# OmerMersin/video-stab

Measured on AMD Instinct MI355X. Metric: stabilized frames/sec @1080p (whole job; warp-stage HBM GB/s in roofline), higher is better.
Workload: dtype u8

## Files before the change

video-stab_amd/csrc/k_pyr.hip:

```cpp
#include "vs_common.h"

namespace vsd {
namespace {

constexpr int NT = 256;
constexpr int RPB = 4;

__global__ __launch_bounds__(NT) void pyr_down_kernel(const uint8_t* __restrict__ src_, size_t sstride,
                                                      int sw, int sh, uint8_t* __restrict__ dst_,
                                                      size_t dstride, int dw, int dh) {
    const uint8_t* __restrict__ src = src_;
    uint8_t* __restrict__ dst = dst_;
    const int x = blockIdx.x * blockDim.x + threadIdx.x;
    if (x >= dw) return;
    int xi[5];
#pragma unroll
    for (int k = 0; k < 5; k++) xi[k] = reflect101(2 * x + k - 2, sw);
    for (int y = blockIdx.y * RPB; y < min((int)(blockIdx.y + 1) * RPB, dh); y++) {
        int col[5];
#pragma unroll
        for (int j = 0; j < 5; j++) {
            const uint8_t* s = src + (size_t)reflect101(2 * y + j - 2, sh) * sstride;
            col[j] = s[xi[2]] * 6 + (s[xi[1]] + s[xi[3]]) * 4 + s[xi[0]] + s[xi[4]];
        }
        dst[(size_t)y * dstride + x] = (uint8_t)((col[2] * 6 + (col[1] + col[3]) * 4 + col[0] + col[4] + 128) >> 8);
    }
}

__global__ __launch_bounds__(NT) void scharr_kernel(const uint8_t* __restrict__ src_, size_t sstride, int w,
                                                    int h, int16_t* __restrict__ dst_) {
    const uint8_t* __restrict__ src = src_;
    int16_t* __restrict__ dst = dst_;
    const int x = blockIdx.x * blockDim.x + threadIdx.x;
    if (x >= w) return;
    for (int y = blockIdx.y * RPB; y < min((int)(blockIdx.y + 1) * RPB, h); y++) {
    const uint8_t* r0 = src + (size_t)(y > 0 ? y - 1 : h > 1 ? 1 : 0) * sstride;
    const uint8_t* r1 = src + (size_t)y * sstride;
    const uint8_t* r2 = src + (size_t)(y < h - 1 ? y + 1 : h > 1 ? h - 2 : 0) * sstride;
    const int xm = x > 0 ? x - 1 : (w > 1 ? 1 : 0);
    const int xp = x < w - 1 ? x + 1 : (w > 1 ? w - 2 : 0);
    const int a_m = (r0[xm] + r2[xm]) * 3 + r1[xm] * 10;
    const int a_p = (r0[xp] + r2[xp]) * 3 + r1[xp] * 10;
    const int b_m = r2[xm] - r0[xm];
    const int b_c = r2[x] - r0[x];
    const int b_p = r2[xp] - r0[xp];
    short2 o;
    o.x = (short)(a_p - a_m);
    o.y = (short)((b_p + b_m) * 3 + b_c * 10);
    *reinterpret_cast<short2*>(dst + ((size_t)y * w + x) * 2) = o;
    }
}

constexpr int FT_W = 64, FT_H = 16;
constexpr int FT_PITCH = 72;
constexpr int FT_ROWS = FT_H + 4;

template <bool DER, bool DOWN>
__global__ __launch_bounds__(NT) void pyr_level_kernel(const ImgPair* __restrict__ sch, const ImgPair* __restrict__ pyr, size_t sstride,
                                                       int w, int h, size_t dstride, int dw, int dh) {
    static_assert(DER || DOWN, "a level launch produces something");
    __shared__ __attribute__((aligned(16))) uint8_t tile[FT_ROWS * FT_PITCH];
    const uint8_t* __restrict__ src = static_cast<const uint8_t*>((DER ? sch : pyr)[blockIdx.z].src);
    const int tid = threadIdx.x;
    const int x0 = blockIdx.x * FT_W, y0 = blockIdx.y * FT_H;
    const bool inside = x0 >= 4 && y0 >= 2 && x0 + FT_W + 4 <= w && y0 + FT_H + 2 <= h && (sstride & 3) == 0 && ((uintptr_t)src & 3) == 0;
    if (inside) {
        constexpr int ND = (FT_ROWS * (FT_PITCH / 4) + NT - 1) / NT;
        uint32_t v[ND];
#pragma unroll
        for (int k = 0; k < ND; k++) {
            const int i = min(tid + NT * k, FT_ROWS * (FT_PITCH / 4) - 1);
            const int r = i / (FT_PITCH / 4), c4 = i - r * (FT_PITCH / 4);
            v[k] = *reinterpret_cast<const uint32_t*>(src + (size_t)(y0 - 2 + r) * sstride + (x0 - 4) + 4 * c4);
        }
#pragma unroll
        for (int k = 0; k < ND; k++)
            if (tid + NT * k < FT_ROWS * (FT_PITCH / 4)) reinterpret_cast<uint32_t*>(tile)[tid + NT * k] = v[k];
    } else if (tid < 3 * FT_PITCH) {
        constexpr int NB = (FT_ROWS + 2) / 3;
        const int c = tid % FT_PITCH, r0 = tid / FT_PITCH;
        const uint8_t* col = src + reflect101(x0 - 4 + c, w);
        size_t off[NB];
#pragma unroll
        for (int k = 0; k < NB; k++) off[k] = (size_t)reflect101(y0 - 2 + min(r0 + 3 * k, FT_ROWS - 1), h) * sstride;
        uint8_t v[NB];
#pragma unroll
        for (int k = 0; k < NB; k++) v[k] = col[off[k]];
#pragma unroll
        for (int k = 0; k < NB; k++)
            if (r0 + 3 * k < FT_ROWS) tile[(r0 + 3 * k) * FT_PITCH + c] = v[k];
    }
    __syncthreads();
    const uint32_t* T = reinterpret_cast<const uint32_t*>(tile);
    if (DER) {
        int16_t* __restrict__ der = static_cast<int16_t*>(sch[blockIdx.z].dst);
        const int r = tid >> 4, c = (tid & 15) * 4;
        const int y = y0 + r, x = x0 + c;
        if (y < h && x < w) {
            int t[3][6];
#pragma unroll
            for (int j = 0; j < 3; j++) {
                const uint32_t* q = T + (r + 1 + j) * (FT_PITCH / 4) + (c >> 2);
                const uint32_t lo = q[0], mid = q[1], hi = q[2];
                t[j][0] = lo >> 24;
                t[j][1] = mid & 255u; t[j][2] = (mid >> 8) & 255u; t[j][3] = (mid >> 16) & 255u; t[j][4] = mid >> 24;
                t[j][5] = hi & 255u;
            }
            int a[6], b[6];
#pragma unroll
            for (int k = 0; k < 6; k++) {
                a[k] = (t[0][k] + t[2][k]) * 3 + t[1][k] * 10;
                b[k] = t[2][k] - t[0][k];
            }
            uint32_t o[4];
#pragma unroll
            for (int k = 0; k < 4; k++) {
                const int dx = a[k + 2] - a[k], dy = (b[k + 2] + b[k]) * 3 + b[k + 1] * 10;
                o[k] = ((uint32_t)dx & 0xFFFFu) | ((uint32_t)dy << 16);
            }
            int16_t* d = der + ((size_t)y * w + x) * 2;
            if (x + 3 < w && (((uintptr_t)d) & 15) == 0) {
                *reinterpret_cast<uint4*>(d) = make_uint4(o[0], o[1], o[2], o[3]);
            } else {
                for (int k = 0; k < 4 && x + k < w; k++) reinterpret_cast<uint32_t*>(d)[k] = o[k];
            }
        }
    }
    if (DOWN) {
        uint8_t* __restrict__ dst = static_cast<uint8_t*>(pyr[blockIdx.z].dst);
        const int xo = (x0 >> 1) + (tid & 31), yo = (y0 >> 1) + (tid >> 5);
        if (xo < dw && yo < dh) {
            const int o = 2 * (tid & 31) + 2, sh = o & 3;
            const uint32_t* q = T + 2 * (tid >> 5) * (FT_PITCH / 4) + (o >> 2);
            int col[5];
#pragma unroll
            for (int j = 0; j < 5; j++) {
                const uint32_t lo = q[j * (FT_PITCH / 4)], hi = q[j * (FT_PITCH / 4) + 1];
                const uint32_t four = __builtin_amdgcn_alignbyte(hi, lo, sh);
                const uint32_t fifth = (hi >> (8 * sh)) & 255u;
                col[j] = (int)__builtin_amdgcn_udot4(four, 0x04060401u, fifth, false);
            }
            dst[(size_t)yo * dstride + xo] = (uint8_t)((col[2] * 6 + (col[1] + col[3]) * 4 + col[0] + col[4] + 128) >> 8);
        }
    }
}

}

int launch_pyr_level_batch(const ImgPair* d_scharr_pairs, const ImgPair* d_pyr_pairs, int items, size_t sstride, int w, int h,
                           size_t dstride, hipStream_t st) {
    if ((!d_scharr_pairs && !d_pyr_pairs) || items < 1 || items > 65535 || w <= 0 || h <= 0 || h > 65535) {
        set_last_error("pyr_level_batch: invalid argument");
        return VS_ERR_INVALID_ARG;
    }
    const int dw = (w + 1) / 2, dh = (h + 1) / 2;
    dim3 grid((w + FT_W - 1) / FT_W, (h + FT_H - 1) / FT_H, items);
    if (!d_scharr_pairs)
        hipLaunchKernelGGL((pyr_level_kernel<false, true>), grid, dim3(NT), 0, st, d_scharr_pairs, d_pyr_pairs, sstride, w, h, dstride, dw, dh);
    else if (d_pyr_pairs)
        hipLaunchKernelGGL((pyr_level_kernel<true, true>), grid, dim3(NT), 0, st, d_scharr_pairs, d_pyr_pairs, sstride, w, h, dstride, dw, dh);
    else hipLaunchKernelGGL((pyr_level_kernel<true, false>), grid, dim3(NT), 0, st, d_scharr_pairs, d_pyr_pairs, sstride, w, h, dstride, dw, dh);
    VS_HIP_TRY(hipGetLastError());
    return VS_OK;
}

int launch_pyr_down(const uint8_t* d_src, size_t sstride, int sw, int sh, uint8_t* d_dst,
                    size_t dstride, hipStream_t st) {
    if (!d_src || !d_dst || sw <= 0 || sh <= 0 || sh > 131070) {
        set_last_error("pyr_down: invalid argument");
        return VS_ERR_INVALID_ARG;
    }
    const int dw = (sw + 1) / 2, dh = (sh + 1) / 2;
    dim3 grid((dw + NT - 1) / NT, (dh + RPB - 1) / RPB);
    hipLaunchKernelGGL(pyr_down_kernel, grid, dim3(NT), 0, st, d_src, sstride, sw, sh, d_dst, dstride, dw, dh);
    VS_HIP_TRY(hipGetLastError());
    return VS_OK;
}

int launch_scharr(const uint8_t* d_src, size_t sstride, int w, int h, int16_t* d_dst, hipStream_t st) {
    if (!d_src || !d_dst || w <= 0 || h <= 0 || h > 65535) {
        set_last_error("scharr: invalid argument");
        return VS_ERR_INVALID_ARG;
    }
    dim3 grid((w + NT - 1) / NT, (h + RPB - 1) / RPB);
    hipLaunchKernelGGL(scharr_kernel, grid, dim3(NT), 0, st, d_src, sstride, w, h, d_dst);
    VS_HIP_TRY(hipGetLastError());
    return VS_OK;
}

}
```

video-stab_amd/csrc/vs_api.cpp:

```cpp
#include <cmath>
#include <cstring>
#include <mutex>
#include <vector>

#include "launchers.h"
#include "vs_common.h"

namespace vsd {

static thread_local std::string g_last_error;
void set_last_error(const std::string& msg) { g_last_error = msg; }
const char* get_last_error() { return g_last_error.c_str(); }

int ensure_device() {
    int n = 0;
    hipError_t e = hipGetDeviceCount(&n);
    if (e != hipSuccess || n <= 0) {
        set_last_error(std::string("no HIP device: ") + (e != hipSuccess ? hipGetErrorString(e) : "count is 0") +
                       " (libvideo-stab has no CPU fallback)");
        return VS_ERR_NO_DEVICE;
    }
    return VS_OK;
}

// ... 149 lines not shown
int vs_dev_sync(void) {
    VS_TRY(ensure_device());
    VS_HIP_TRY(hipDeviceSynchronize());
    return VS_OK;
}
int vs_dev_memcpy_d2d(void* d_dst, const void* d_src, size_t bytes) {
    VS_TRY(ensure_device());
    VS_HIP_TRY(hipMemcpy(d_dst, d_src, bytes, hipMemcpyDeviceToDevice));
    return VS_OK;
}
int vs_op_libm_checksum(int fn, uint64_t start, uint64_t count, uint64_t* result) {
    if (fn < 0 || fn > 3 || !result || count == 0) return VS_ERR_INVALID_ARG;
    VS_TRY(ensure_device());
    return vsd::run_libm_checksum(fn, start, count, result);
}
int vs_dev_copy_rate(size_t bytes, int iters, double* gbytes_per_s) {
    if (!gbytes_per_s || bytes < 4096 || iters < 1 || iters > 1000) return VS_ERR_INVALID_ARG;
    VS_TRY(ensure_device());
    return vsd::run_copy_rate(bytes, iters, gbytes_per_s);
}

int vs_op_warp_affine(const void* d_src, size_t src_stride, size_t src_frame_bytes, void* d_dst,
                      size_t dst_stride, size_t dst_frame_bytes, int w, int h, int cn,
                      const float* M, int batch, void* stream) {
    VS_TRY(ensure_device());
    if (!d_src || !d_dst || !M || batch <= 0) { set_last_error("warp_affine: invalid argument"); return VS_ERR_INVALID_ARG; }
    std::vector<double> Minv(6 * (size_t)batch);
    for (int b = 0; b < batch; b++) warp_invert(M + 6 * (size_t)b, &Minv[6 * (size_t)b]);
    const auto srcs = frame_list((const uint8_t*)d_src, src_frame_bytes, batch);
    const auto dsts = frame_list((uint8_t*)d_dst, dst_frame_bytes, batch);
    return launch_warp_plane(srcs.data(), dsts.data(), batch, src_stride, w, h, dst_stride, w, h, cn, WarpMaps{Minv.data(), 6, true},
                             VS_BORDER_BLACK, WarpTabs{WarpTabs::SCRATCH}, (hipStream_t)stream);
}

static int warp_affine_two_planes(const void* d_src, size_t src_stride, void* d_dst, size_t dst_stride, int w, int h, const float* M, int batch,
                                  size_t src_frame_bytes, size_t dst_frame_bytes, void* stream, int sample_bytes) {
    VS_TRY(ensure_device());
    if (!d_src || !d_dst || !M || batch <= 0) {
        set_last_error(sample_bytes == 2 ? "warp_affine_p010: invalid argument" : "warp_affine_nv12: invalid argument");
        return VS_ERR_INVALID_ARG;
    }
    if (sample_bytes == 2 && ((src_frame_bytes | dst_frame_bytes) & 1)) {
        set_last_error("warp_affine_p010: frame distances must be even (16-bit samples)");
        return VS_ERR_INVALID_ARG;
    }
    std::vector<double> Minv(12 * (size_t)batch);
    for (int b = 0; b < batch; b++) {
        const float* m = M + 6 * (size_t)b;
        const float c[6] = {m[0], m[1], m[2] * 0.5f, m[3], m[4], m[5] * 0.5f};
        warp_invert(m, &Minv[12 * (size_t)b]);
        warp_invert(c, &Minv[12 * (size_t)b + 6]);
    }
    const size_t suv = (size_t)h * src_stride, duv = (size_t)h * dst_stride;
    const auto ys = frame_list((const uint8_t*)d_src, src_frame_bytes, batch), us = frame_list((const uint8_t*)d_src, src_frame_bytes, batch, suv);
    const auto yd = frame_list((uint8_t*)d_dst, dst_frame_bytes, batch), ud = frame_list((uint8_t*)d_dst, dst_frame_bytes, batch, duv);
    return launch_warp_nv12(ys.data(), yd.data(), us.data(), ud.data(), batch, src_stride, dst_stride, w, h, WarpMaps{Minv.data(), 12, true},
                            VS_BORDER_BLACK, WarpTabs{WarpTabs::SCRATCH}, (hipStream_t)stream, sample_bytes);
}

int vs_op_warp_affine_nv12(const void* d_src, size_t src_stride, void* d_dst, size_t dst_stride,
                           int w, int h, const float* M, int batch, size_t src_frame_bytes,
                           size_t dst_frame_bytes, void* stream) {
    return warp_affine_two_planes(d_src, src_stride, d_dst, dst_stride, w, h, M, batch, src_frame_bytes, dst_frame_bytes, stream, 1);
}

int vs_op_warp_affine_p010(const void* d_src, size_t src_stride, void* d_dst, size_t dst_stride,
                           int w, int h, const float* M, int batch, size_t src_frame_bytes,
                           size_t dst_frame_bytes, void* stream) {
    return warp_affine_two_planes(d_src, src_stride, d_dst, dst_stride, w, h, M, batch, src_frame_bytes, dst_frame_bytes, stream, 2);
}

static int warp_affine_three_planes(const void* d_src, size_t src_stride, size_t src_u_off, size_t src_v_off, size_t src_c_pitch, void* d_dst,
                                    size_t dst_stride, size_t dst_u_off, size_t dst_v_off, size_t dst_c_pitch, int w, int h, const float* M, int batch,
                                    size_t src_frame_bytes, size_t dst_frame_bytes, int border, void* stream, int sample_bytes, int sx = 1, int sy = 1) {
    VS_TRY(ensure_device());
    const size_t half = sx ? 2 * (size_t)sample_bytes - 1 : 0;
    if (!d_src || !d_dst || !M || batch <= 0 || w < 1 || h < 1 || (w >> sx) < 1 || (h >> sy) < 1 || (w & ((1 << sx) - 1)) || (h & ((1 << sy) - 1)) ||
        (!src_c_pitch && (src_stride & half)) || (!dst_c_pitch && (dst_stride & half))) {
        if (sy == 0) set_last_error(sx ? "warp_affine_planar: 4:2:2: invalid argument (w must be even and, for the default chroma pitch, the strides hold two chroma rows)"
                                       : "warp_affine_planar: 4:4:4: invalid argument");
        else set_last_error(sample_bytes == 2 ? "warp_affine_i010: invalid argument (w and h must be even and, for the default chroma pitch, the strides multiples of 4)"
                                              : "warp_affine_i420: invalid argument (w, h and, for the default chroma pitch, the strides must be even)");
        return VS_ERR_INVALID_ARG;
    }
    if (sample_bytes == 2 && ((src_frame_bytes | dst_frame_bytes) & 1)) {
        set_last_error(sy == 0 ? "warp_affine_planar: frame distances must be even (16-bit samples)" : "warp_affine_i010: frame distances must be even (16-bit samples)");
        return VS_ERR_INVALID_ARG;
    }
    std::vector<double> Minv(12 * (size_t)batch);
    for (int b = 0; b < batch; b++) {
        const float* m = M + 6 * (size_t)b;
        float c[6] = {m[0], m[1], m[2] * 0.5f, m[3], m[4], m[5] * 0.5f};
        if (sx == 1 && sy == 0) { c[1] = m[1] * 0.5f; c[3] = m[3] * 2.0f; c[5] = m[5]; }
        else if (sx == 0) { c[2] = m[2]; c[5] = m[5]; }
        warp_invert(m, &Minv[12 * (size_t)b]);
        warp_invert(c, &Minv[12 * (size_t)b + 6]);
    }
    const I420Layout sl = i420_layout(src_stride, h, src_u_off, src_v_off, src_c_pitch, sx, sy), dl = i420_layout(dst_stride, h, dst_u_off, dst_v_off, dst_c_pitch, sx, sy);
    const auto ys = frame_list((const uint8_t*)d_src, src_frame_bytes, batch);
    const auto yd = frame_list((uint8_t*)d_dst, dst_frame_bytes, batch);
    return launch_warp_i420(ys.data(), yd.data(), batch, sl, dl, w, h, WarpMaps{Minv.data(), 12, true}, border, WarpTabs{WarpTabs::SCRATCH},
                            (hipStream_t)stream, sample_bytes, sx, sy);
}

int vs_op_warp_affine_i420(const void* d_src, size_t src_stride, size_t src_u_off, size_t src_v_off, size_t src_c_pitch, void* d_dst, size_t dst_stride,
                           size_t dst_u_off, size_t dst_v_off, size_t dst_c_pitch, int w, int h, const float* M, int batch, size_t src_frame_bytes,
                           size_t dst_frame_bytes, int border, void* stream) {
    return warp_affine_three_planes(d_src, src_stride, src_u_off, src_v_off, src_c_pitch, d_dst, dst_stride, dst_u_off, dst_v_off, dst_c_pitch, w, h, M,
                                    batch, src_frame_bytes, dst_frame_bytes, border, stream, 1);
}

int vs_op_warp_affine_i010(const void* d_src, size_t src_stride, size_t src_u_off, size_t src_v_off, size_t src_c_pitch, void* d_dst, size_t dst_stride,
                           size_t dst_u_off, size_t dst_v_off, size_t dst_c_pitch, int w, int h, const float* M, int batch, size_t src_frame_bytes,
                           size_t dst_frame_bytes, int border, void* stream) {
    return warp_affine_three_planes(d_src, src_stride, src_u_off, src_v_off, src_c_pitch, d_dst, dst_stride, dst_u_off, dst_v_off, dst_c_pitch, w, h, M,
                                    batch, src_frame_bytes, dst_frame_bytes, border, stream, 2);
}

int vs_op_warp_affine_planar(int fmt, const void* d_src, size_t src_stride, size_t src_u_off, size_t src_v_off, size_t src_c_pitch, void* d_dst,
                             size_t dst_stride, size_t dst_u_off, size_t dst_v_off, size_t dst_c_pitch, int w, int h, const float* M, int batch,
                             size_t src_frame_bytes, size_t dst_frame_bytes, int border, void* stream) {
    const PixFmt* pf = pixfmt(fmt);
    if (!pf || !pf->three_planes()) {
        VS_TRY(ensure_device());
        set_last_error("warp_affine_planar: fmt must be a planar format (VS_FMT_I420 ... VS_FMT_I412)");
        return VS_ERR_INVALID_ARG;
    }
    return warp_affine_three_planes(d_src, src_stride, src_u_off, src_v_off, src_c_pitch, d_dst, dst_stride, dst_u_off, dst_v_off, dst_c_pitch, w, h, M,
                                    batch, src_frame_bytes, dst_frame_bytes, border, stream, pf->sample_bytes, pf->sx, pf->sy);
}

int vs_op_resize_gray(const void* d_src, size_t src_stride, int sw, int sh, int fmt, void* d_dst,
                      size_t dst_stride, int dw, int dh, void* stream) {
    VS_TRY(ensure_device());
    return launch_resize_gray((const uint8_t*)d_src, src_stride, sw, sh, fmt, (uint8_t*)d_dst,
                              dst_stride, dw, dh, (hipStream_t)stream);
}

int vs_op_pyr_down(const void* d_src, size_t src_stride, int sw, int sh, void* d_dst,
                   size_t dst_stride, void* stream) {
    VS_TRY(ensure_device());
    return launch_pyr_down((const uint8_t*)d_src, src_stride, sw, sh, (uint8_t*)d_dst, dst_stride,
                           (hipStream_t)stream);
}

int vs_op_scharr(const void* d_src, size_t src_stride, int w, int h, void* d_dst, void* stream) {
    VS_TRY(ensure_device());
    return launch_scharr((const uint8_t*)d_src, src_stride, w, h, (int16_t*)d_dst, (hipStream_t)stream);
}

int vs_op_pyr_level(const void* d_src, size_t src_stride, size_t src_frame_bytes, int w, int h, void* d_der, void* d_next,
                    size_t next_stride, size_t next_frame_bytes, int items, void* stream) {
    VS_TRY(ensure_device());
    if (!d_src || !d_der || items < 1 || items > 4096 || w <= 0 || h <= 0) { set_last_error("pyr_level: invalid argument"); return VS_ERR_INVALID_ARG; }
    std::vector<ImgPair> t(2 * (size_t)items);
    for (int i = 0; i < items; i++) {
        const uint8_t* s = (const uint8_t*)d_src + (size_t)i * src_frame_bytes;
        t[i] = ImgPair{s, (uint8_t*)d_der + (size_t)i * w * h * 4};
        t[items + i] = ImgPair{s, d_next ? (uint8_t*)d_next + (size_t)i * next_frame_bytes : nullptr};
    }
    ImgPair* d_t = nullptr;
    VS_HIP_TRY(hipMalloc((void**)&d_t, sizeof(ImgPair) * t.size()));
    hipStream_t st = (hipStream_t)stream;
    int rc = VS_OK;
    if (hipMemcpyAsync(d_t, t.data(), sizeof(ImgPair) * t.size(), hipMemcpyHostToDevice, st) != hipSuccess) rc = VS_ERR_HIP;
    if (rc == VS_OK) rc = launch_pyr_level_batch(d_t, d_next ? d_t + items : nullptr, items, src_stride, w, h, next_stride, st);
    (void)hipStreamSynchronize(st);
    (void)hipFree(d_t);
    return rc;
}

int vs_op_pyr_lk(const void* d_prev, const void* d_next, size_t stride, int w, int h,
                 const float* d_prev_pts, int n, float* d_next_pts, uint8_t* d_status, float* d_err,
                 int win, int max_level, int max_iters, double eps, void* stream) {
    VS_TRY(ensure_device());
    return run_pyr_lk_op((const uint8_t*)d_prev, (const uint8_t*)d_next, stride, w, h, d_prev_pts, n,
                         d_next_pts, d_status, d_err, win, max_level, max_iters, eps,
                         (hipStream_t)stream);
}

int vs_op_gftt(const void* d_gray, size_t stride, int w, int h, int max_corners, double quality,
               double min_distance, int block_size, float* d_pts, int32_t* d_count, float* d_eig,
               void* stream) {
    VS_TRY(ensure_device());
    return run_gftt_op((const uint8_t*)d_gray, stride, w, h, max_corners, quality, min_distance,
                       block_size, d_pts, d_count, d_eig, (hipStream_t)stream);
}

int vs_op_estimate_affine_partial2d(const float* d_from, const float* d_to, int n, double thr,
                                    int max_iters, double* d_model, uint8_t* d_inliers,
                                    int32_t* d_info, void* stream) {
    VS_TRY(ensure_device());
    return run_estimate_affine_partial2d(d_from, d_to, n, thr, max_iters, d_model, d_inliers, d_info,
                                         (hipStream_t)stream);
}

}
```

video-stab_amd/vsamd/capi.py:

```python
import collections
import ctypes as C
import os

import numpy as np

PKG_DIR = os.path.dirname(os.path.dirname(os.path.abspath(__file__)))
LIB_PATH = os.path.join(PKG_DIR, "csrc", "libvideo-stab.so")

u8p = C.POINTER(C.c_uint8)
f32p = C.POINTER(C.c_float)
f64p = C.POINTER(C.c_double)
i32p = C.POINTER(C.c_int32)

PixFmt = collections.namedtuple("PixFmt", "fmt name text kind cn sample_bytes bits sx sy gray_source border_modes")
KIND_INTERLEAVED, KIND_LUMA_UV, KIND_THREE_PLANES = range(3)
PIXFMTS = (
    PixFmt(0, "BGR8", "BGR8", KIND_INTERLEAVED, 3, 1, 8, 0, 0, 0, True),
    PixFmt(1, "NV12", "NV12", KIND_LUMA_UV, 1, 1, 8, 1, 1, 2, False),
    PixFmt(2, "GRAY8", "GRAY8", KIND_INTERLEAVED, 1, 1, 8, 0, 0, 2, False),
    PixFmt(3, "BGRA8", "BGRA8", KIND_INTERLEAVED, 4, 1, 8, 0, 0, 3, True),
    PixFmt(4, "RGBA8", "RGBA8", KIND_INTERLEAVED, 4, 1, 8, 0, 0, 4, True),
    PixFmt(5, "RGB8", "RGB8", KIND_INTERLEAVED, 3, 1, 8, 0, 0, 5, True),
    PixFmt(6, "P010", "P010", KIND_LUMA_UV, 2, 2, 10, 1, 1, 6, False),
    PixFmt(7, "I420", "I420", KIND_THREE_PLANES, 1, 1, 8, 1, 1, 2, False),
# ... 453 lines not shown
            assert hasattr(p, k), k
            setattr(p, k, v)
        return p

    def sync(self):
        self.check(self.lib.vs_dev_sync())

    def trajectory(self, params, streams, steps=None):
        n = len(streams)
        mods = [np.ascontiguousarray(m, np.float64).reshape(-1, 6) for m, _ in streams]
        kinds = [np.ascontiguousarray(k, np.int32) for _, k in streams]
        npush = (C.c_int32 * n)(*[len(k) for k in kinds])
        dbg = [(VsDebugFrame * (2 * len(k) + 2))() for k in kinds]
        rel = [(VsTrajRelease * (len(k) + 1))() for k in kinds]
        n_dbg, n_rel = (C.c_int32 * n)(), (C.c_int32 * n)()
        mp = (C.POINTER(C.c_double) * n)(*[m.ctypes.data_as(C.POINTER(C.c_double)) for m in mods])
        kp = (C.POINTER(C.c_int32) * n)(*[k.ctypes.data_as(C.POINTER(C.c_int32)) for k in kinds])
        dp = (C.POINTER(VsDebugFrame) * n)(*[C.cast(d, C.POINTER(VsDebugFrame)) for d in dbg])
        rp = (C.POINTER(VsTrajRelease) * n)(*[C.cast(r, C.POINTER(VsTrajRelease)) for r in rel])
        st = (C.c_int32 * len(steps))(*steps) if steps else None
        self.check(self.lib.vs_op_trajectory(C.byref(params), n, mp, kp, npush, 0 if steps is None else 1, st, len(steps) if steps else 0,
                                             dp, n_dbg, rp, n_rel))
        return [(list(dbg[s][:n_dbg[s]]), list(rel[s][:n_rel[s]])) for s in range(n)]

    def warp_affine(self, img, M, batch=None):
        img = np.ascontiguousarray(img)
        batched = img.ndim == 4 or (img.ndim == 3 and (img.shape[2] not in (1, 3) if batch is None else batch))
        if img.ndim == 2:
            b, (h, w), cn = 1, img.shape, 1
        elif img.ndim == 3 and not batched:
            b, (h, w, cn) = 1, img.shape
        elif img.ndim == 3:
            (b, h, w), cn = img.shape, 1
        else:
            b, h, w, cn = img.shape
        M = np.ascontiguousarray(M, np.float32).reshape(b, 6)
        d_in = DevBuf.from_array(self, img)
        d_out = DevBuf(self, img.nbytes)
        fb = h * w * cn
        self.check(self.lib.vs_op_warp_affine(d_in.ptr, w * cn, fb, d_out.ptr, w * cn, fb, w, h, cn,
                                              _p(M, f32p), b, None))
        self.sync()
        return d_out.download(img.shape, np.uint8)

    def warp_affine_nv12(self, img, w, h, M):
        img = np.ascontiguousarray(img)
        M = np.ascontiguousarray(M, np.float32).reshape(-1, 6)
        n = M.shape[0]
        fb = img.nbytes // n
        d_in = DevBuf.from_array(self, img)
        d_out = DevBuf(self, img.nbytes)
        self.check(self.lib.vs_op_warp_affine_nv12(d_in.ptr, w, d_out.ptr, w, w, h, _p(M, f32p), n, fb, fb, None))
        self.sync()
        return d_out.download(img.shape, np.uint8)

    def warp_affine_p010(self, img, w, h, M):
        img = np.ascontiguousarray(img, np.uint16)
        M = np.ascontiguousarray(M, np.float32).reshape(-1, 6)
        n = M.shape[0]
        fb = img.nbytes // n
        d_in = DevBuf.from_array(self, img)
        d_out = DevBuf(self, img.nbytes)
        self.check(self.lib.vs_op_warp_affine_p010(d_in.ptr, 2 * w, d_out.ptr, 2 * w, w, h, _p(M, f32p), n, fb, fb, None))
        self.sync()
        return d_out.download(img.shape, np.uint16)

    def warp_affine_i420(self, img, w, h, M, border=BORDER_BLACK):
        img = np.ascontiguousarray(img, np.uint8)
        M = np.ascontiguousarray(M, np.float32).reshape(-1, 6)
        n = M.shape[0]
        fb = img.nbytes // n
        d_in = DevBuf.from_array(self, img)
        d_out = DevBuf(self, img.nbytes)
        try:
            self.check(self.lib.vs_op_warp_affine_i420(d_in.ptr, w, 0, 0, 0, d_out.ptr, w, 0, 0, 0, w, h, _p(M, f32p), n, fb, fb, border, None))
            self.sync()
            return d_out.download(img.shape, np.uint8)
        finally:
            d_in.free(); d_out.free()

    def warp_affine_i010(self, img, w, h, M, border=BORDER_BLACK):
        img = np.ascontiguousarray(img, np.uint16)
        M = np.ascontiguousarray(M, np.float32).reshape(-1, 6)
        n = M.shape[0]
        fb = img.nbytes // n
        d_in = DevBuf.from_array(self, img)
        d_out = DevBuf(self, img.nbytes)
        try:
            self.check(self.lib.vs_op_warp_affine_i010(d_in.ptr, 2 * w, 0, 0, 0, d_out.ptr, 2 * w, 0, 0, 0, w, h, _p(M, f32p), n, fb, fb, border, None))
            self.sync()
            return d_out.download(img.shape, np.uint16)
        finally:
            d_in.free(); d_out.free()

    def warp_affine_planar(self, fmt, img, w, h, M, border=BORDER_BLACK):
        dt = fmt_dtype(fmt)
        img = np.ascontiguousarray(img, dt)
        M = np.ascontiguousarray(M, np.float32).reshape(-1, 6)
        n = M.shape[0]
        fb = img.nbytes // n
        sb = fmt_px_bytes(fmt)
        d_in = DevBuf.from_array(self, img)
        d_out = DevBuf(self, img.nbytes)
        try:
            self.check(self.lib.vs_op_warp_affine_planar(fmt, d_in.ptr, sb * w, 0, 0, 0, d_out.ptr, sb * w, 0, 0, 0, w, h, _p(M, f32p), n, fb, fb, border, None))
            self.sync()
            return d_out.download(img.shape, dt)
        finally:
            d_in.free(); d_out.free()

    def resize_gray(self, img, dw, dh, fmt=None):
        img = np.ascontiguousarray(img)
        if fmt is None:
            fmt = FMT_BGR8 if img.ndim == 3 else FMT_GRAY8
        w = img.shape[1]
        h = img.shape[0] if not fmt_two_planes(fmt) else img.shape[0] * 2 // 3
        cn = fmt_px_bytes(fmt)
        d_in = DevBuf.from_array(self, img)
        d_out = DevBuf(self, dw * dh)
        self.check(self.lib.vs_op_resize_gray(d_in.ptr, w * cn, w, h, fmt, d_out.ptr, dw, dw, dh, None))
        self.sync()
        return d_out.download((dh, dw), np.uint8)

    def pyr_down(self, g):
        g = np.ascontiguousarray(g)
        h, w = g.shape
        dh, dw = (h + 1) // 2, (w + 1) // 2
        d_in = DevBuf.from_array(self, g)
        d_out = DevBuf(self, dw * dh)
        self.check(self.lib.vs_op_pyr_down(d_in.ptr, w, w, h, d_out.ptr, dw, None))
        self.sync()
        return d_out.download((dh, dw), np.uint8)

    def scharr(self, g):
        g = np.ascontiguousarray(g)
        h, w = g.shape
        d_in = DevBuf.from_array(self, g)
        d_out = DevBuf(self, h * w * 4)
        self.check(self.lib.vs_op_scharr(d_in.ptr, w, w, h, d_out.ptr, None))
        self.sync()
        return d_out.download((h, w, 2), np.int16)

    def pyr_level(self, g, down=True):
        g = np.ascontiguousarray(g)
        h, w = g.shape
        dh, dw = (h + 1) // 2, (w + 1) // 2
        d_in = DevBuf.from_array(self, g)
        d_der = DevBuf(self, h * w * 4)
        d_next = DevBuf(self, dw * dh) if down else None
        self.check(self.lib.vs_op_pyr_level(d_in.ptr, w, w * h, w, h, d_der.ptr, d_next.ptr if down else None, dw, dw * dh, 1, None))
        self.sync()
        return d_der.download((h, w, 2), np.int16), (d_next.download((dh, dw), np.uint8) if down else None)

    def pyr_lk(self, prev, nxt, pts, win=15, max_level=2, iters=20, eps=0.03):
        prev = np.ascontiguousarray(prev)
        nxt = np.ascontiguousarray(nxt)
        pts = np.ascontiguousarray(pts, np.float32).reshape(-1, 2)
        n = pts.shape[0]
        h, w = prev.shape
        d_prev = DevBuf.from_array(self, prev)
        d_next = DevBuf.from_array(self, nxt)
        d_pts = DevBuf.from_array(self, pts)
        d_out = DevBuf(self, n * 8)
        d_st = DevBuf(self, n)
        d_err = DevBuf(self, n * 4)
        self.check(self.lib.vs_op_pyr_lk(d_prev.ptr, d_next.ptr, w, w, h, d_pts.ptr, n, d_out.ptr, d_st.ptr,
                                         d_err.ptr, win, max_level, iters, eps, None))
        self.sync()
        return (d_out.download((n, 2), np.float32), d_st.download((n,), np.uint8),
                d_err.download((n,), np.float32))

    def gftt(self, g, max_corners, quality, min_distance, block_size=3, want_eig=False):
        g = np.ascontiguousarray(g)
        h, w = g.shape
        d_in = DevBuf.from_array(self, g)
        d_pts = DevBuf(self, max(max_corners, 1) * 8)
        d_cnt = DevBuf(self, 16)
        d_eig = DevBuf(self, w * h * 4) if want_eig else None
        self.check(self.lib.vs_op_gftt(d_in.ptr, w, w, h, max_corners, quality, min_distance, block_size,
                                       d_pts.ptr, d_cnt.ptr, d_eig.ptr if d_eig else None, None))
        self.sync()
        n = int(d_cnt.download((1,), np.int32)[0])
        pts = d_pts.download((max(max_corners, 1), 2), np.float32)[:n].copy()
        if want_eig:
            return pts, d_eig.download((h, w), np.float32)
        return pts

    def estimate_affine_partial2d(self, a, b, thr=5.0, max_iters=500):
        a = np.ascontiguousarray(a, np.float32).reshape(-1, 2)
        b = np.ascontiguousarray(b, np.float32).reshape(-1, 2)
        n = a.shape[0]
        d_a = DevBuf.from_array(self, a)
        d_b = DevBuf.from_array(self, b)
        d_model = DevBuf(self, 48)
        d_inl = DevBuf(self, max(n, 1))
        d_info = DevBuf(self, 16)
        self.check(self.lib.vs_op_estimate_affine_partial2d(d_a.ptr, d_b.ptr, n, thr, max_iters, d_model.ptr,
                                                            d_inl.ptr, d_info.ptr, None))
        self.sync()
        info = d_info.download((4,), np.int32)
        return (int(info[0]), d_model.download((6,), np.float64), d_inl.download((max(n, 1),), np.uint8)[:n], info)

    def canny(self, g, low, high):
        g = np.ascontiguousarray(g)
        h, w = g.shape
        d_in = DevBuf.from_array(self, g)
        d_out = DevBuf(self, w * h)
        self.check(self.lib.vs_op_canny(d_in.ptr, w, w, h, low, high, d_out.ptr, w, None))
        self.sync()
        return d_out.download((h, w), np.uint8)

    def hough_lines(self, edges, rho, theta, threshold, max_lines=8192):
        edges = np.ascontiguousarray(edges)
        h, w = edges.shape
        d_in = DevBuf.from_array(self, edges)
        d_lines = DevBuf(self, max_lines * 8)
        d_cnt = DevBuf(self, 16)
        self.check(self.lib.vs_op_hough_lines(d_in.ptr, w, w, h, rho, theta, threshold, d_lines.ptr, max_lines,
                                              d_cnt.ptr, None))
        self.sync()
        n = int(d_cnt.download((1,), np.int32)[0])
        return d_lines.download((max_lines, 2), np.float32)[:n].copy()

    def warp_affine_ex(self, img, M, border=BORDER_BLACK, dsize=None):
        img = np.ascontiguousarray(img)
        h, w = img.shape[:2]
        cn = 1 if img.ndim == 2 else img.shape[2]
        dw, dh = dsize if dsize else (w, h)
        M = np.ascontiguousarray(M, np.float64).reshape(6)
        d_in = DevBuf.from_array(self, img)
        d_out = DevBuf(self, dw * dh * cn)
        self.check(self.lib.vs_op_warp_affine_ex(d_in.ptr, w * cn, w, h, d_out.ptr, dw * cn, dw, dh, cn,
                                                 _p(M, f64p), border, None))
        self.sync()
        return d_out.download((dh, dw) if img.ndim == 2 else (dh, dw, cn), np.uint8)

    def warp_affine16_ex(self, img, M, border=BORDER_BLACK, dsize=None):
        img = np.ascontiguousarray(img, np.uint16)
        h, w = img.shape[:2]
        cn = 1 if img.ndim == 2 else img.shape[2]
        dw, dh = dsize if dsize else (w, h)
        M = np.ascontiguousarray(M, np.float64).reshape(6)
        d_in = DevBuf.from_array(self, img)
        d_out = DevBuf(self, dw * dh * cn * 2)
        self.check(self.lib.vs_op_warp_affine16_ex(d_in.ptr, w * cn * 2, w, h, d_out.ptr, dw * cn * 2, dw, dh, cn,
                                                   _p(M, f64p), border, None))
        self.sync()
        return d_out.download((dh, dw) if img.ndim == 2 else (dh, dw, cn), np.uint16)

    @staticmethod
    def _scale_job_array(jobs):
        arr = (VsScaleJob * max(1, len(jobs)))()
        for i, (src, src_stride, sw, sh, dst, dst_stride, dw, dh, cn) in enumerate(jobs):
            arr[i] = VsScaleJob(src, src_stride, sw, sh, dst, dst_stride, dw, dh, cn, 0)
        return arr

    def scale_jobs(self, jobs, sample_bytes=1, path=0, stream=None):
        self.check(self.lib.vs_op_scale_jobs(self._scale_job_array(jobs), len(jobs), sample_bytes, path, stream))

    def scale_jobs_plan(self, jobs, sample_bytes=1):
        staged = np.zeros(max(1, len(jobs)), np.int32)
        self.check(self.lib.vs_op_scale_jobs_plan(self._scale_job_array(jobs), len(jobs), sample_bytes, _p(staged, i32p)))
        return staged[:len(jobs)].copy()

    def copy_make_border(self, img, b, border, src_pitch=None):
        img = np.ascontiguousarray(img, np.uint8)
        h, w = img.shape[:2]
        cn = 1 if img.ndim == 2 else img.shape[2]
        pitch = src_pitch or w * cn
        rows = np.full((h, pitch), 0xA5, np.uint8)
        rows[:, :w * cn] = img.reshape(h, w * cn)
        ow, oh = w + 2 * b, h + 2 * b
        d_in = DevBuf.from_array(self, rows)
        d_out = DevBuf(self, ow * oh * cn)
        self.check(self.lib.vs_op_copy_make_border(d_in.ptr, pitch, w, h, cn, d_out.ptr, ow * cn, b, border, None))
        self.sync()
        return d_out.download((oh, ow) if img.ndim == 2 else (oh, ow, cn), np.uint8)

    def fade_blend(self, hist, frame, alpha, beta):
        hist = np.ascontiguousarray(hist, np.uint8).reshape(-1)
        frame = np.ascontiguousarray(frame, np.uint8).reshape(-1)
        assert hist.size == frame.size
        pad = (-hist.size) % 4
        d_h = DevBuf.from_array(self, np.concatenate([hist, np.zeros(pad, np.uint8)]))
        d_f = DevBuf.from_array(self, np.concatenate([frame, np.zeros(pad, np.uint8)]))
        self.check(self.lib.vs_op_fade_blend(d_h.ptr, d_f.ptr, hist.size, alpha, beta, None))
        self.sync()
        return d_f.download((hist.size,), np.uint8)

    def fade_update(self, hist, stab, row_bytes, rows):
        hist = np.ascontiguousarray(hist, np.uint8).reshape(-1)
        stab = np.ascontiguousarray(stab, np.uint8)
        assert stab.shape[0] == rows and stab.shape[1] >= row_bytes and hist.size >= rows * row_bytes
        d_h = DevBuf.from_array(self, hist)
        d_s = DevBuf.from_array(self, stab)
        self.check(self.lib.vs_op_fade_update(d_h.ptr, d_s.ptr, stab.shape[1], row_bytes, rows, None))
        self.sync()
        return d_h.download((hist.size,), np.uint8)

    def cvt_coefficients(self, colorimetry=None):
        out = np.zeros(16, np.int32)
        self.check(self.lib.vs_cvt_coefficients(_cs_ref(colorimetry), _p(out, i32p)))
        return out

    def cvt_colorimetry_guess(self, w, h):
        cs = CvtColorimetry(-1, -1, -1, -1)
# ... 814 lines not shown
```

Baseline: 131,700.

## Add register-strip pyramid downsample kernel for downsample-only levels

```diff
diff --git a/scratch/pyr_launches.py b/scratch/pyr_launches.py
--- /dev/null
+++ b/scratch/pyr_launches.py
@@ -0,0 +1,27 @@
+import collections, csv, glob, statistics, sys
+
+d = sys.argv[1]
+label = sys.argv[2] if len(sys.argv) > 2 else d
+names = ("pyr_level_kernel", "pyr_next_kernel", "pyr_next_px_kernel")
+dur = collections.defaultdict(dict)
+for f in glob.glob(d + "/**/*kernel_trace.csv", recursive=True):
+    for r in csv.DictReader(open(f)):
+        k = next((n for n in names if n + "(" in r["Kernel_Name"] or n + "<" in r["Kernel_Name"]), None)
+        if k:
+            grid = tuple(int(r.get("Grid_Size_" + a) or 0) for a in "XYZ")
+            dur[(k, grid)][int(r["Dispatch_Id"])] = int(r["End_Timestamp"]) - int(r["Start_Timestamp"])
+cnt = collections.defaultdict(lambda: collections.defaultdict(float))
+for f in glob.glob(d + "/**/*counter_collection.csv", recursive=True):
+    for r in csv.DictReader(open(f)):
+        cnt[int(r["Dispatch_Id"])][r["Counter_Name"]] += float(r["Counter_Value"])
+print("== %s" % label)
+for (k, grid), v in sorted(dur.items(), key=lambda kv: -kv[0][1][0] * kv[0][1][1] * kv[0][1][2]):
+    ids = sorted(v)
+    ids = ids[len(ids) // 4:]
+    us = sorted(v[i] / 1e3 for i in ids)
+    q = lambda p: us[min(len(us) - 1, int(p * len(us)))]
+    print("%s grid %dx%dx%d n=%4d  median %7.1f us  p10 %7.1f  p90 %7.1f  min %7.1f  max %7.1f" %
+          ((k,) + grid + (len(us), statistics.median(us), q(0.1), q(0.9), us[0], us[-1])))
+    cs = sorted(set(c for i in ids for c in cnt.get(i, {})))
+    if cs:
+        print("  " + "  ".join("%s=%.0f" % (c, statistics.mean(cnt[i][c] for i in ids if i in cnt)) for c in cs))
diff --git a/video-stab_amd/csrc/k_pyr.hip b/video-stab_amd/csrc/k_pyr.hip
--- a/video-stab_amd/csrc/k_pyr.hip
+++ b/video-stab_amd/csrc/k_pyr.hip
@@ -145,6 +145,133 @@
     }
 }
 
+constexpr int PN_R = 4;
+constexpr int PN_ROWS = 2 * PN_R + 3;
+typedef uint32_t pn_u32x4 __attribute__((ext_vector_type(4)));
+typedef pn_u32x4 pn_u32x4_a4 __attribute__((aligned(4)));
+#define PN_GLOBAL __attribute__((address_space(1)))
+
+__device__ __forceinline__ uint8_t pyr_next_px(const uint8_t* __restrict__ src, size_t sstride, int w, int h, int xo, int yo) {
+    int xi[5];
+    size_t ro[5];
+#pragma unroll
+    for (int k = 0; k < 5; k++) {
+        xi[k] = reflect101(2 * xo + k - 2, w);
+        ro[k] = (size_t)reflect101(2 * yo + k - 2, h) * sstride;
+    }
+    uint8_t v[5][5];
+#pragma unroll
+    for (int j = 0; j < 5; j++)
+#pragma unroll
+        for (int k = 0; k < 5; k++) v[j][k] = src[ro[j] + xi[k]];
+    int col[5];
+#pragma unroll
+    for (int j = 0; j < 5; j++) col[j] = v[j][2] * 6 + (v[j][1] + v[j][3]) * 4 + v[j][0] + v[j][4];
+    return (uint8_t)((col[2] * 6 + (col[1] + col[3]) * 4 + col[0] + col[4] + 128) >> 8);
+}
+
+__global__ __launch_bounds__(NT) void pyr_next_px_kernel(const ImgPair* __restrict__ pyr, size_t sstride, int w, int h, size_t dstride,
+                                                         int dw, int dh) {
+    const uint8_t* __restrict__ src = static_cast<const uint8_t*>(pyr[blockIdx.z].src);
+    uint8_t* __restrict__ dst = static_cast<uint8_t*>(pyr[blockIdx.z].dst);
+    const uint32_t idx = blockIdx.x * NT + threadIdx.x;
+    const int yo = (int)(idx / (uint32_t)dw), xo = (int)(idx - (uint32_t)yo * (uint32_t)dw);
+    if (yo >= dh) return;
+    dst[(size_t)yo * dstride + xo] = pyr_next_px(src, sstride, w, h, xo, yo);
+}
+
+__global__ __launch_bounds__(NT) void pyr_next_kernel(const ImgPair* __restrict__ pyr, uint32_t sstride, int w, int h, uint32_t dstride,
+                                                      int dw, int dh, int ni, int n_in, int n_in_pad, int strips) {
+    const uint8_t* __restrict__ src = static_cast<const uint8_t*>(pyr[blockIdx.z].src);
+    uint8_t* __restrict__ dst = static_cast<uint8_t*>(pyr[blockIdx.z].dst);
+    const int idx = blockIdx.x * NT + threadIdx.x;
+    int g, strip;
+    if (idx < n_in) {
+        strip = idx / ni;
+        g = idx - strip * ni + 1;
+    } else {
+        const int e = idx - n_in_pad;
+        if (e < 0 || e >= 2 * strips) return;
+        strip = e >> 1;
+        g = (e & 1) ? ni + 1 : 0;
+    }
+    const int y0 = strip * PN_R;
+    if ((uintptr_t)src & 3) {
+#pragma unroll 1
+        for (int k = 0; k < 4 * PN_R; k++) {
+            const int xo = 4 * g + (k & 3), yo = y0 + (k >> 2);
+            if (xo < dw && yo < dh) dst[(size_t)yo * dstride + xo] = pyr_next_px(src, sstride, w, h, xo, yo);
+        }
+        return;
+    }
+    const PN_GLOBAL uint8_t* gsrc = (const PN_GLOBAL uint8_t*)src;
+    PN_GLOBAL uint8_t* gdst = (PN_GLOBAL uint8_t*)dst;
+    const int s0 = 8 * g - 4;
+    const int cs = min(max(s0, 0), w - 16);
+    const int shift = (s0 - cs) >> 2;
+    const int r0 = 2 * y0 - 2;
+    uint32_t off[PN_ROWS];
+    if (r0 >= 0 && r0 + PN_ROWS <= h) {
+#pragma unroll
+        for (int j = 0; j < PN_ROWS; j++) off[j] = (uint32_t)(r0 + j) * sstride + (uint32_t)cs;
+    } else {
+#pragma unroll
+        for (int j = 0; j < PN_ROWS; j++) {
+            const int a = abs(r0 + j);
+            off[j] = (uint32_t)max(min(a, 2 * h - 2 - a), 0) * sstride + (uint32_t)cs;
+        }
+    }
+    pn_u32x4 v[PN_ROWS];
+#pragma unroll
+    for (int j = 0; j < PN_ROWS; j++) v[j] = *reinterpret_cast<const PN_GLOBAL pn_u32x4_a4*>(gsrc + off[j]);
+    if (shift < 0) {
+#pragma unroll
+        for (int j = 0; j < PN_ROWS; j++) {
+            const pn_u32x4 a = v[j];
+            v[j].x = (a.x & 0x00FF0000u) | ((a.x & 0x0000FF00u) << 16); v[j].y = a.x; v[j].z = a.y; v[j].w = a.z;
+        }
+    } else if (shift == 1) {
+#pragma unroll
+        for (int j = 0; j < PN_ROWS; j++) {
+            const pn_u32x4 a = v[j];
+            v[j].x = a.y; v[j].y = a.z; v[j].z = a.w; v[j].w = a.w >> 16;
+        }
+    } else if (shift == 2) {
+#pragma unroll
+        for (int j = 0; j < PN_ROWS; j++) {
+            const pn_u32x4 a = v[j];
+            v[j].x = a.z; v[j].y = a.w; v[j].z = a.w >> 16;
+        }
+    }
+    uint32_t hs[PN_ROWS][4];
+#pragma unroll
+    for (int j = 0; j < PN_ROWS; j++) {
+        const uint32_t b = v[j].y, c = v[j].z;
+        hs[j][0] = __builtin_amdgcn_udot4(__builtin_amdgcn_alignbyte(b, v[j].x, 2), 0x04060401u, (b >> 16) & 255u, false);
+        hs[j][1] = __builtin_amdgcn_udot4(b, 0x04060401u, c & 255u, false);
+        hs[j][2] = __builtin_amdgcn_udot4(__builtin_amdgcn_alignbyte(c, b, 2), 0x04060401u, (c >> 16) & 255u, false);
+        hs[j][3] = __builtin_amdgcn_udot4(c, 0x04060401u, v[j].w & 255u, false);
+    }
+    const bool dwords = 4 * g + 3 < dw && (((uintptr_t)dst | dstride) & 3) == 0;
+    uint32_t doff = (uint32_t)y0 * dstride + 4u * (uint32_t)g;
+#pragma unroll
+    for (int r = 0; r < PN_R; r++, doff += dstride) {
+        if (y0 + r >= dh) break;
+        uint32_t s[4];
+#pragma unroll
+        for (int i = 0; i < 4; i++)
+            s[i] = __umul24(hs[2 * r + 2][i], 6u) + ((hs[2 * r + 1][i] + hs[2 * r + 3][i]) << 2) + (hs[2 * r][i] + hs[2 * r + 4][i] + 128u);
+        const uint32_t o = __builtin_amdgcn_perm(s[1], s[0], 0x0C0C0501u) | __builtin_amdgcn_perm(s[3], s[2], 0x05010C0Cu);
+        if (dwords) {
+            *reinterpret_cast<PN_GLOBAL uint32_t*>(gdst + doff) = o;
+        } else {
+#pragma unroll
+            for (int i = 0; i < 4; i++)
+                if (4 * g + i < dw) gdst[doff + i] = (uint8_t)(o >> (8 * i));
+        }
+    }
+}
+
 }
 
 int launch_pyr_level_batch(const ImgPair* d_scharr_pairs, const ImgPair* d_pyr_pairs, int items, size_t sstride, int w, int h,
@@ -155,9 +282,27 @@
     }
     const int dw = (w + 1) / 2, dh = (h + 1) / 2;
     dim3 grid((w + FT_W - 1) / FT_W, (h + FT_H - 1) / FT_H, items);
-    if (!d_scharr_pairs)
-        hipLaunchKernelGGL((pyr_level_kernel<false, true>), grid, dim3(NT), 0, st, d_scharr_pairs, d_pyr_pairs, sstride, w, h, dstride, dw, dh);
-    else if (d_pyr_pairs)
+    if (!d_scharr_pairs) {
+        if ((sstride & 3) == 0 && (w & 3) == 0 && w >= 16 && h >= 3 && (uint64_t)h * sstride <= 0xFFFFFFFFull &&
+            (uint64_t)dh * dstride <= 0xFFFFFFFFull) {
+            const int ni = (dw + 3) / 4 - 2, strips = (dh + PN_R - 1) / PN_R;
+            const int64_t n_in = (int64_t)ni * strips, n_in_pad = (n_in + 63) / 64 * 64, lanes = n_in_pad + 2 * strips;
+            if (lanes > INT32_MAX - NT) {
+                set_last_error("pyr_level_batch: image too large");
+                return VS_ERR_INVALID_ARG;
+            }
+            hipLaunchKernelGGL(pyr_next_kernel, dim3((unsigned)((lanes + NT - 1) / NT), 1, items), dim3(NT), 0, st, d_pyr_pairs, (uint32_t)sstride, w, h,
+                               (uint32_t)dstride, dw, dh, ni, (int)n_in, (int)n_in_pad, strips);
+        } else {
+            const int64_t lanes = (int64_t)dw * dh;
+            if (lanes > INT32_MAX - NT) {
+                set_last_error("pyr_level_batch: image too large");
+                return VS_ERR_INVALID_ARG;
+            }
+            hipLaunchKernelGGL(pyr_next_px_kernel, dim3((unsigned)((lanes + NT - 1) / NT), 1, items), dim3(NT), 0, st, d_pyr_pairs, sstride, w, h,
+                               dstride, dw, dh);
+        }
+    } else if (d_pyr_pairs)
         hipLaunchKernelGGL((pyr_level_kernel<true, true>), grid, dim3(NT), 0, st, d_scharr_pairs, d_pyr_pairs, sstride, w, h, dstride, dw, dh);
     else hipLaunchKernelGGL((pyr_level_kernel<true, false>), grid, dim3(NT), 0, st, d_scharr_pairs, d_pyr_pairs, sstride, w, h, dstride, dw, dh);
     VS_HIP_TRY(hipGetLastError());
diff --git a/video-stab_amd/csrc/vs_api.cpp b/video-stab_amd/csrc/vs_api.cpp
--- a/video-stab_amd/csrc/vs_api.cpp
+++ b/video-stab_amd/csrc/vs_api.cpp
@@ -325,11 +325,11 @@
 int vs_op_pyr_level(const void* d_src, size_t src_stride, size_t src_frame_bytes, int w, int h, void* d_der, void* d_next,
                     size_t next_stride, size_t next_frame_bytes, int items, void* stream) {
     VS_TRY(ensure_device());
-    if (!d_src || !d_der || items < 1 || items > 4096 || w <= 0 || h <= 0) { set_last_error("pyr_level: invalid argument"); return VS_ERR_INVALID_ARG; }
+    if (!d_src || (!d_der && !d_next) || items < 1 || items > 4096 || w <= 0 || h <= 0) { set_last_error("pyr_level: invalid argument"); return VS_ERR_INVALID_ARG; }
     std::vector<ImgPair> t(2 * (size_t)items);
     for (int i = 0; i < items; i++) {
         const uint8_t* s = (const uint8_t*)d_src + (size_t)i * src_frame_bytes;
-        t[i] = ImgPair{s, (uint8_t*)d_der + (size_t)i * w * h * 4};
+        t[i] = ImgPair{s, d_der ? (uint8_t*)d_der + (size_t)i * w * h * 4 : nullptr};
         t[items + i] = ImgPair{s, d_next ? (uint8_t*)d_next + (size_t)i * next_frame_bytes : nullptr};
     }
     ImgPair* d_t = nullptr;
@@ -337,7 +337,7 @@
     hipStream_t st = (hipStream_t)stream;
     int rc = VS_OK;
     if (hipMemcpyAsync(d_t, t.data(), sizeof(ImgPair) * t.size(), hipMemcpyHostToDevice, st) != hipSuccess) rc = VS_ERR_HIP;
-    if (rc == VS_OK) rc = launch_pyr_level_batch(d_t, d_next ? d_t + items : nullptr, items, src_stride, w, h, next_stride, st);
+    if (rc == VS_OK) rc = launch_pyr_level_batch(d_der ? d_t : nullptr, d_next ? d_t + items : nullptr, items, src_stride, w, h, next_stride, st);
     (void)hipStreamSynchronize(st);
     (void)hipFree(d_t);
     return rc;
diff --git a/video-stab_amd/vsamd/capi.py b/video-stab_amd/vsamd/capi.py
--- a/video-stab_amd/vsamd/capi.py
+++ b/video-stab_amd/vsamd/capi.py
@@ -629,6 +629,27 @@
         self.sync()
         return d_der.download((h, w, 2), np.int16), (d_next.download((dh, dw), np.uint8) if down else None)
 
+    def pyr_next(self, imgs, src_pitch=None, dst_pitch=None, src_offset=0, fill=0xA5):
+        imgs = np.ascontiguousarray(imgs, np.uint8)
+        if imgs.ndim == 2:
+            imgs = imgs[None]
+        n, h, w = imgs.shape
+        dh, dw = (h + 1) // 2, (w + 1) // 2
+        sp = w if src_pitch is None else int(src_pitch)
+        dp = dw if dst_pitch is None else int(dst_pitch)
+        assert sp >= w and dp >= dw
+        src = np.full((n, h, sp), 0x5A, np.uint8)
+        src[:, :, :w] = imgs
+        d_in = DevBuf(self, src_offset + src.nbytes)
+        d_out = DevBuf.from_array(self, np.full((n, dh, dp), fill, np.uint8))
+        try:
+            d_in.upload(src, src_offset)
+            self.check(self.lib.vs_op_pyr_level(d_in.ptr + src_offset, sp, h * sp, w, h, None, d_out.ptr, dp, dh * dp, n, None))
+            self.sync()
+            return d_out.download((n, dh, dp), np.uint8)
+        finally:
+            d_in.free(); d_out.free()
+
     def pyr_lk(self, prev, nxt, pts, win=15, max_level=2, iters=20, eps=0.03):
         prev = np.ascontiguousarray(prev)
         nxt = np.ascontiguousarray(nxt)
```

Result: no change. 133,800, median of 6 (+1.5%).
